# Decade-qiu/Go2NetSpectra

Hardware: AMD Instinct MI355X
Metric: Mpackets/s CMS update (device-resident, d=4 w=2^20) at 1/2/4/8 MI355X (higher is better)
Workload: dtype u32; 1 GPU; configs[1]: Count-Min d=4 w=2^20, 100M Zipf(1.1) 5-tuple headers in HBM per GPU, bit-exact counters; device_batch=100000000, key=5-tuple (37 B), parallelism=owner-key shards x1 (SrcIP slot; each GPU generates its shard of the stream), windows=steps use stream windows 0..619 (warmup first), none replayed

## Files before the change

go2netspectra_amd/_lib.py:

```python
from __future__ import annotations

import ctypes as ct
import os
import subprocess

_HERE = os.path.dirname(os.path.abspath(__file__))
LIB_PATH = os.environ.get("GNS_LIB") or os.path.join(_HERE, "libgns_sketch.so")
CSRC = os.path.join(_HERE, "csrc")

GNS_OK = 0
GNS_E_ARG, GNS_E_HIP, GNS_E_OOM, GNS_E_FULL, GNS_E_RANGE, GNS_E_NODEV = -1, -2, -3, -4, -5, -6
ERRORS = {-1: "GNS_E_ARG", -2: "GNS_E_HIP", -3: "GNS_E_OOM", -4: "GNS_E_FULL", -5: "GNS_E_RANGE",
          -6: "GNS_E_NODEV"}
MEM_HOST, MEM_DEVICE = 0, 1

FIELD_IDS = {"SrcIP": 1, "DstIP": 2, "SrcPort": 3, "DstPort": 4, "Protocol": 5}
FIELD_NAMES = {v: k for k, v in FIELD_IDS.items()}
FIELD_SIZE = {"SrcIP": 16, "DstIP": 16, "SrcPort": 2, "DstPort": 2, "Protocol": 1}

EXPORTED = [
    "gns_cm_create", "gns_cm_destroy", "gns_cm_insert_keys", "gns_cm_insert_tuples",
    "gns_cm_insert_headers", "gns_cm_flush", "gns_cm_query", "gns_cm_query_device", "gns_cm_heavy_hitters", "gns_cm_reset",
    "gns_cm_export_state", "gns_cm_stats", "gns_cm_counters", "gns_cm_set_timing", "gns_cm_stage_times", "gns_cm_stream",
    "gns_cm_view_create", "gns_cm_view_destroy", "gns_cm_view_refresh", "gns_cm_view_heavy_hitters",
    "gns_cm_view_query",
    "gns_ss_create", "gns_ss_destroy", "gns_ss_insert_keys", "gns_ss_insert_tuples",
    "gns_ss_insert_headers", "gns_ss_flush", "gns_ss_query", "gns_ss_query_device", "gns_ss_heavy_hitters", "gns_ss_reset",
    "gns_ss_export_state", "gns_ss_stats", "gns_ss_counters", "gns_ss_set_timing", "gns_ss_stage_times",
    "gns_synth_create", "gns_synth_destroy", "gns_synth_fill", "gns_synth_flows",
    "gns_ex_create", "gns_ex_destroy", "gns_ex_insert_tuples", "gns_ex_insert_headers", "gns_ex_flush",
    "gns_ex_query", "gns_ex_query_device", "gns_ex_snapshot", "gns_ex_reset", "gns_ex_counters", "gns_ex_set_timing",
    "gns_ex_stage_times",
    "gns_thrift_decode", "gns_pack_pcap", "gns_pack_pcap_ts", "gns_pack_counts", "gns_frame_record", "gns_last_error", "gns_version",
    "gns_route_create", "gns_route_destroy", "gns_route_partition",
    "gns_cm_dict_stats", "gns_ss_dict_stats", "gns_ex_dict_stats", "gns_cm_reclaim", "gns_ss_reclaim",
    "gns_cm_insert_compact", "gns_pack_pcap_compact", "gns_compact_headers", "gns_route_partition_async",
    "gns_pack_pcap_compact16", "gns_compact_headers16",
    "gns_route_owner_fields", "gns_route_create_keyed", "gns_route_owner_layout", "gns_route_owner_keys",
    "gns_device_alloc", "gns_device_free", "gns_cm_heavy_rows", "gns_hh_order_rows",
    "gns_exs_create", "gns_exs_destroy", "gns_exs_insert_keys", "gns_exs_insert_tuples", "gns_exs_insert_headers",
    "gns_exs_flush", "gns_exs_query", "gns_exs_query_device", "gns_exs_heavy_hitters", "gns_exs_snapshot",
    "gns_exs_reset", "gns_exs_counters", "gns_exs_dict_stats", "gns_exs_set_timing", "gns_exs_stage_times",
    "gns_ex_aggregate", "gns_ex_heavy_hitters",
    "gns_ex_view_create", "gns_ex_view_destroy", "gns_ex_view_refresh", "gns_ex_view_snapshot",
    "gns_ex_view_aggregate", "gns_ex_view_heavy_hitters",
    "gns_pairs_export", "gns_pairs_merge", "gns_pairs_merge_from",
    "gns_ss_insert_compact", "gns_spread_insert_compact", "gns_ex_insert_compact", "gns_pack_pcap_compact_ts",
    "gns_ss_view_create", "gns_ss_view_destroy", "gns_ss_view_refresh", "gns_ss_view_query",
    "gns_ss_view_query_device", "gns_ss_view_heavy_hitters", "gns_ss_view_heavy_rows", "gns_ss_view_export_state",
    "gns_cm_view_refresh_at", "gns_cm_view_query_device", "gns_cm_view_heavy_rows", "gns_cm_view_export_state",
    "gns_ex_rollup", "gns_spread_rollup",
    "gns_ex_rollup_prefix", "gns_spread_rollup_prefix", "gns_ex_aggregate_cidr", "gns_ex_view_aggregate_cidr",
    "gns_ex_hist_create", "gns_ex_hist_destroy", "gns_ex_hist_append", "gns_ex_hist_times", "gns_ex_hist_stats",
    "gns_ex_hist_aggregate", "gns_ex_hist_aggregate_cidr", "gns_ex_hist_heavy_hitters", "gns_ex_hist_snapshot",
    "gns_ex_hist_trim", "gns_ex_hist_export", "gns_ex_hist_append_rows",
    "gns_hh_hist_create", "gns_hh_hist_destroy", "gns_hh_hist_append", "gns_hh_hist_heavy_hitters",
    "gns_hh_hist_heavy_rows", "gns_hh_hist_times", "gns_hh_hist_stats", "gns_hh_hist_export",
]


class GnsError(RuntimeError):
    def __init__(self, code: int, msg: str):
        super().__init__(f"{ERRORS.get(code, code)}: {msg}")
        self.code = code


class Layout(ct.Structure):
    _fields_ = [("n_fields", ct.c_uint32), ("fields", ct.c_uint8 * 8)]

    @classmethod
    def of(cls, fields) -> "Layout":
        fields = list(fields or [])
        if len(fields) > 8:
            raise ValueError("at most 8 key fields")
        lay = cls()
        lay.n_fields = len(fields)
        for i, f in enumerate(fields):
            lay.fields[i] = FIELD_IDS.get(f, 0)
        return lay

    def names(self):
        return [FIELD_NAMES.get(int(self.fields[i]), "") for i in range(self.n_fields)]


class Tuples(ct.Structure):
    _fields_ = [("src16", ct.c_void_p), ("dst16", ct.c_void_p), ("sport", ct.c_void_p),
                ("dport", ct.c_void_p), ("proto", ct.c_void_p), ("length", ct.c_void_p)]


class CmParams(ct.Structure):
# ... 92 lines not shown
        "gns_cm_stream": ([vp], vp),
        "gns_cm_view_create": ([vp, vp], i32), "gns_cm_view_destroy": ([vp], i32),
        "gns_cm_view_refresh": ([vp], i32), "gns_cm_view_heavy_hitters": ([vp, vp, vp, vp, vp, vp, vp], i32),
        "gns_cm_view_query": ([vp, vp, u32, u64, vp], i32),
        "gns_ss_create": ([vp, vp], i32), "gns_ss_destroy": ([vp], i32),
        "gns_ss_insert_keys": ([vp, vp, u32, vp, u32, u64, i32], i32),
        "gns_ss_insert_tuples": ([vp, vp, u64, i32], i32),
        "gns_ss_insert_headers": ([vp, vp, vp, u64, i32], i32),
        "gns_ss_flush": ([vp], i32), "gns_ss_query": ([vp, vp, u32, u64, vp], i32),
        "gns_ss_query_device": ([vp, vp, u32, u64, vp], i32),
        "gns_ss_heavy_hitters": ([vp, vp, vp, vp], i32), "gns_ss_reset": ([vp], i32),
        "gns_ss_export_state": ([vp, vp, vp, vp, vp], i32), "gns_ss_stats": ([vp, vp], i32),
        "gns_ss_counters": ([vp, vp], i32),
        "gns_ss_set_timing": ([vp, i32], i32), "gns_ss_stage_times": ([vp, vp, vp, i32], i32),
        "gns_synth_create": ([vp, vp], i32), "gns_synth_destroy": ([vp], i32),
        "gns_synth_fill": ([vp, vp, vp, u64, u64], i32), "gns_synth_flows": ([vp, vp], i32),
        "gns_ex_create": ([vp, vp], i32), "gns_ex_destroy": ([vp], i32),
        "gns_ex_insert_tuples": ([vp, vp, vp, vp, u64, i32], i32),
        "gns_ex_insert_headers": ([vp, vp, vp, vp, u64, i32], i32),
        "gns_ex_flush": ([vp], i32), "gns_ex_query": ([vp, vp, u32, u64, vp], i32),
        "gns_ex_query_device": ([vp, vp, u32, u64, vp], i32),
        "gns_ex_snapshot": ([vp, vp, vp, vp, vp, vp, vp], i32), "gns_ex_reset": ([vp], i32),
        "gns_ex_counters": ([vp, vp], i32), "gns_ex_set_timing": ([vp, i32], i32),
        "gns_ex_stage_times": ([vp, vp, vp, i32], i32),
        "gns_thrift_decode": ([vp, u64, vp, u64, vp, vp, vp, vp, i32, i32], i32),
        "gns_pack_pcap": ([ct.c_char_p, vp, vp, u64, vp], ct.c_int64),
        "gns_pack_pcap_ts": ([ct.c_char_p, vp, vp, vp, u64, vp], ct.c_int64),
        "gns_pack_counts": ([vp], ct.c_int),
        "gns_frame_record": ([vp, ct.c_uint32, ct.c_uint32, vp], ct.c_int),
        "gns_last_error": ([], ct.c_char_p), "gns_version": ([], ct.c_char_p),
        "gns_route_create": ([u32, i32, vp], i32), "gns_route_destroy": ([vp], i32),
        "gns_route_partition": ([vp, vp, vp, u64, vp, vp, vp], i32),
        "gns_cm_dict_stats": ([vp, vp], i32), "gns_ss_dict_stats": ([vp, vp], i32),
        "gns_ex_dict_stats": ([vp, vp], i32), "gns_cm_reclaim": ([vp], i32), "gns_ss_reclaim": ([vp], i32),
        "gns_cm_insert_compact": ([vp, vp, vp, u64, vp, u64, i32], i32),
        "gns_pack_pcap_compact": ([ct.c_char_p, vp, vp, u64, vp, u64, vp, vp], ct.c_int64),
        "gns_compact_headers": ([vp, vp, u64, vp, vp, u64, vp, i32], i32),
        "gns_pack_pcap_compact16": ([ct.c_char_p, vp, u64, vp, u64, vp, vp], ct.c_int64),
        "gns_compact_headers16": ([vp, vp, u64, vp, vp, u64, vp, i32], i32),
        "gns_route_partition_async": ([vp, vp, vp, u64, vp, vp, vp, vp], i32),
        "gns_route_owner_fields": ([vp, u32, vp], i32),
        "gns_route_create_keyed": ([u32, vp, i32, vp], i32),
        "gns_route_owner_layout": ([vp, vp], i32),
        "gns_route_owner_keys": ([vp, vp, vp, u32, u64, vp, i32], i32),
        "gns_device_alloc": ([u64, i32, vp], i32), "gns_device_free": ([vp, i32], i32),
        "gns_cm_heavy_rows": ([vp, vp, vp, vp, vp], i32),
        "gns_hh_order_rows": ([vp, u32, u64, vp, i32], i32),
        "gns_exs_create": ([vp, vp], i32), "gns_exs_destroy": ([vp], i32),
        "gns_exs_insert_keys": ([vp, vp, u32, vp, u32, u64, i32], i32),
        "gns_exs_insert_tuples": ([vp, vp, u64, i32], i32),
        "gns_exs_insert_headers": ([vp, vp, vp, u64, i32], i32),
        "gns_exs_flush": ([vp], i32), "gns_exs_query": ([vp, vp, u32, u64, vp], i32),
        "gns_exs_query_device": ([vp, vp, u32, u64, vp], i32),
        "gns_exs_heavy_hitters": ([vp, u32, vp, vp, vp], i32), "gns_exs_snapshot": ([vp, vp, vp, vp], i32),
        "gns_exs_reset": ([vp], i32), "gns_exs_counters": ([vp, vp], i32), "gns_exs_dict_stats": ([vp, vp], i32),
        "gns_exs_set_timing": ([vp, i32], i32), "gns_exs_stage_times": ([vp, vp, vp, i32], i32),
        "gns_ex_aggregate": ([vp, vp, u32, vp], i32),
        "gns_ex_heavy_hitters": ([vp, i32, u64, u64, vp, vp, vp], i32),
        "gns_cm_import_state": ([vp, vp, vp, vp, vp, vp], i32),
        "gns_ss_import_state": ([vp, vp, vp, vp, vp, u64, vp], i32),
        "gns_ex_merge": ([vp, vp, vp, vp, vp, vp, u64, i32], i32),
        "gns_ex_rollup": ([vp, vp, vp], i32),
        "gns_spread_rollup": ([vp, vp, u64, vp, vp], i32),
        "gns_ex_rollup_prefix": ([vp, vp, vp, vp], i32),
        "gns_spread_rollup_prefix": ([vp, vp, vp, vp, u64, vp, vp], i32),
        "gns_ex_aggregate_cidr": ([vp, vp, u32, vp], i32),
# ... 113 lines not shown
```

go2netspectra_amd/csrc/gns_cm.hip:

```cpp
#include <algorithm>
#include <atomic>
#include <cstdlib>
#include <mutex>
#include <vector>

#include "gns_coldmask.cuh"
#include "gns_common.hpp"
#include "gns_ctl.cuh"
#include "gns_hh.hpp"
#include "gns_scan.cuh"
#include "gns_xcd.cuh"

namespace gns {

#ifndef GNS_TILE_BITS
#define GNS_TILE_BITS 12
#endif
#ifndef GNS_AP_THREADS
#define GNS_AP_THREADS 1024
#endif
#ifndef GNS_AP_ITEMS
#define GNS_AP_ITEMS 8
#endif
constexpr uint32_t kTileBitsMax = GNS_TILE_BITS;
// ... 2516 lines not shown
    uint32_t *C = nullptr, *S = nullptr, *Fc = nullptr, *Fs = nullptr;
    CmRead rd;
    std::atomic<uint32_t> period{0};
    std::mutex views_mu;
    std::vector<gns_cm_view *> views;
    uint32_t epoch = 0;
    uint64_t bmax = 0;
    uint32_t nblk_max = 0;
    uint32_t *keyid = nullptr, *idx = nullptr;
    uint64_t *cold = nullptr;
    uint64_t *pend[2] = {nullptr, nullptr};
    uint32_t *pcnt[2] = {nullptr, nullptr};
    uint32_t *ptotal = nullptr;
    uint32_t *hist = nullptr, *part = nullptr, *total = nullptr, *order = nullptr;
    uint64_t *entries = nullptr;
    uint64_t *ovf = nullptr;
    uint32_t *ovf_cnt = nullptr;
    uint64_t ovf_cap = 0;
    unsigned long long *stats = nullptr;
    uint32_t *hot_ids = nullptr;
    uint32_t *hot_tab = nullptr;
    long long *segtot = nullptr;
    uint32_t *hflag = nullptr, *hhist = nullptr, *hthr = nullptr, *hcnt = nullptr;
    uint32_t *hcand = nullptr, *hcn = nullptr;
    HotSum *hsum = nullptr;
    uint32_t *hflag2 = nullptr;
    uint32_t *work = nullptr;
    uint32_t ncu = 256;
    uint32_t *hres = nullptr;
    uint4 *chk = nullptr;
    bool warm = false;
    bool lds_ordered = false;
    uint32_t *h_pin = nullptr;
    HostStage stage[2];
    CompactInput compact;
    hipStream_t cstream = nullptr;
    hipEvent_t ev_copied[2] = {nullptr, nullptr}, ev_used[2] = {nullptr, nullptr};
    StageTimer timer;
};

enum : uint32_t { kViewPlain = 0, kViewDetached = 1 };
constexpr uint64_t kCmvPiece = 1u << 18;

struct gns_cm_view : ViewCore {
    gns_cm *cm = nullptr;
    uint32_t *C = nullptr, *S = nullptr, *Fc = nullptr, *Fs = nullptr;
    CmRead rd;
    uint32_t period = ~0u;
    std::atomic<uint32_t> kind{kViewPlain};
    DictDev T{};
    uint64_t tab_cap = 0;
    uint32_t *remap = nullptr;
    uint64_t remap_n = 0;
    uint32_t *scan = nullptr;
    uint64_t scan_n = 0;
    uint32_t *words = nullptr;
    unsigned long long *ctr = nullptr;
    uint8_t *xbytes = nullptr;
    uint64_t xbytes_n = 0;
    PinnedOut po;
    uint32_t *hsm = nullptr;
};

struct ViewsQuiesced {
    std::unique_lock<std::mutex> reg;
    std::vector<std::unique_lock<std::mutex>> locks;
    explicit ViewsQuiesced(gns_cm *cm) : reg(cm->views_mu) {
        locks.reserve(cm->views.size());
        for (gns_cm_view *v : cm->views)
            if (v->kind.load() != kViewDetached) locks.emplace_back(v->mu);
    }
};

namespace {

int cm_free_all(gns_cm *cm) {
    dfree(cm->C); dfree(cm->S); dfree(cm->Fc); dfree(cm->Fs); cm->rd.free_all();
    dfree(cm->keyid); dfree(cm->idx); dfree(cm->cold);
    dfree(cm->pend[0]); dfree(cm->pend[1]); dfree(cm->pcnt[0]); dfree(cm->pcnt[1]);
    dfree(cm->ptotal); dfree(cm->hist); dfree(cm->part); dfree(cm->total); dfree(cm->order);
    dfree(cm->entries); dfree(cm->ovf); dfree(cm->ovf_cnt); dfree(cm->stats);
    cm->stage[0].free_all(); cm->stage[1].free_all(); cm->compact.free_all();
    for (int i = 0; i < 2; i++) {
        if (cm->ev_copied[i]) (void)hipEventDestroy(cm->ev_copied[i]);
        if (cm->ev_used[i]) (void)hipEventDestroy(cm->ev_used[i]);
    }
    if (cm->cstream) (void)hipStreamDestroy(cm->cstream);
    dfree(cm->work);
    dfree(cm->hot_ids); dfree(cm->segtot); dfree(cm->hflag); dfree(cm->hhist); dfree(cm->hthr); dfree(cm->hcnt);
    dfree(cm->hcand); dfree(cm->hcn);
    dfree(cm->hsum); dfree(cm->hflag2); dfree(cm->hres); dfree(cm->chk); dfree(cm->hot_tab);
    cm->FlowDict::free_all();
    if (cm->h_pin) (void)hipHostFree(cm->h_pin);
    cm->timer.destroy();
    if (cm->stream) (void)hipStreamDestroy(cm->stream);
    return GNS_OK;
}

int cm_reset_state(gns_cm *cm) {
    const uint64_t cells = (uint64_t)cm->g.d * cm->g.w;
    GNS_HIP(hipMemsetAsync(cm->C, 0, cells * 4, cm->stream));
    GNS_HIP(hipMemsetAsync(cm->S, 0, cells * 4, cm->stream));
    GNS_HIP(hipMemsetAsync(cm->Fc, 0xFF, cells * 4, cm->stream));
    GNS_HIP(hipMemsetAsync(cm->Fs, 0xFF, cells * 4, cm->stream));
    GNS_HIP(hipMemsetAsync(cm->D.rec, 0, cm->dict_slots * cm->D.RW * 4, cm->stream));
    GNS_HIP(hipMemsetAsync(cm->hot_ids, 0xFF, (size_t)cm->g.d * kHot * 4, cm->stream));
    GNS_HIP(hipMemsetAsync(cm->hot_tab, 0xFF, (size_t)cm->g.d * kHotTab * 4, cm->stream));
    GNS_HIP(hipMemsetAsync(cm->hhist, 0, (size_t)cm->g.d * kHotKeys * 4, cm->stream));
    GNS_HIP(hipMemsetAsync(cm->hthr, 0xFF, 8 * 4, cm->stream));
    GNS_HIP(hipMemsetAsync(cm->hcn, 0, 16 * 4, cm->stream));
    GNS_HIP(hipMemsetAsync(cm->stats + 3, 0, 2 * sizeof(unsigned long long), cm->stream));
    GNS_HIP(hipMemsetAsync(cm->dctl, 0, 16, cm->stream));
    cm->claimed = 0;
    cm->full = false;
    cm->warm = false;
    return GNS_OK;
}

int cm_reclaim(gns_cm *cm, uint64_t min_slots = 0) {
    ViewsQuiesced q(cm);
    const uint64_t cells = (uint64_t)cm->g.d * cm->g.w;
    std::vector<DictIds> ids{{cm->Fc, cells}, {cm->Fs, cells}};
    const uint32_t period = cm->period.load();
    for (gns_cm_view *v : cm->views)
        if (v->kind.load() != kViewDetached && v->period == period) {
            ids.push_back({v->Fc, cells});
            ids.push_back({v->Fs, cells});
        }
    return cm->reclaim(ids.data(), (int)ids.size(), min_slots, cm->stream);
}

template <int KIND, int MODE>
int cm_run_batch(gns_cm *cm, const InputDesc &in, uint64_t n) {
    if (n == 0) return GNS_OK;
    hipStream_t s = cm->stream;
    const uint32_t nblk = (uint32_t)((n + kChunk - 1) / kChunk);
    const CmGeom &g = cm->g;
    ScopedStage total_stage(cm->timer, 5);
    {
        CtlZero z;
        z.add(cm->ptotal, 8);
        z.add(cm->dctl + 1, 4);
        z.add(cm->hflag2, ((size_t)g.d * kHot + 2) * 4);
        z.add(cm->stats + 8, 8);
        z.add(cm->ovf_cnt, 4);
        z.add(cm->work, 4);
        z.add(cm->hflag, (size_t)g.d * kHot * 4);
        GNS_HIP(ctl_zero(z, s));
// ... 5 lines not shown
        a.keyid = cm->keyid; a.idx = cm->idx; a.cold = cm->cold; a.pend = cm->pend[0]; a.pend_cnt = cm->pcnt[0];
        a.pend_total = cm->ptotal; a.hist = cm->hist; a.nblk = nblk; a.hot_ids = cm->hot_ids;
        a.Fc = cm->Fc; a.Fs = cm->Fs; a.hsum = cm->hsum; a.hot_tab = cm->hot_tab;
        a.stats = cm->stats;
        ScopedStage st(cm->timer, 0);
        const size_t lds = extract_lds_bytes(g.nbins_all, g.d);
        if constexpr (KIND == IN_REC16) {
            if (lds > kExLdsSmall)
                hipLaunchKernelGGL((k_extract<KIND, MODE, 0, 0, 1024>), dim3(nblk), dim3(1024), lds, s, a);
            else
                hipLaunchKernelGGL((k_extract<KIND, MODE, 0, 0, 256>), dim3(nblk), dim3(kExThreads), lds, s, a);
        } else if (lds > kExLdsSmall) {
            if (cm->K == 37 && g.d == 8)
                hipLaunchKernelGGL((k_extract<KIND, MODE, 37, 8, kC5Threads>), dim3(nblk), dim3(kC5Threads), lds, s, a);
            else if (cm->K == 37)
                hipLaunchKernelGGL((k_extract<KIND, MODE, 37, 0, 1024>), dim3(nblk), dim3(1024), lds, s, a);
            else if (cm->K == 16)
                hipLaunchKernelGGL((k_extract<KIND, MODE, 16, 0, 1024>), dim3(nblk), dim3(1024), lds, s, a);
            else
                hipLaunchKernelGGL((k_extract<KIND, MODE, 0, 0, 1024>), dim3(nblk), dim3(1024), lds, s, a);
        } else if (cm->K == 37 && g.d == 4)
            hipLaunchKernelGGL((k_extract<KIND, MODE, 37, 4, 256>), dim3(nblk), dim3(kExThreads), lds, s, a);
        else if (cm->K == 37)
            hipLaunchKernelGGL((k_extract<KIND, MODE, 37, 0, 256>), dim3(nblk), dim3(kExThreads), lds, s, a);
        else if (cm->K == 16 && g.d == 4)
            hipLaunchKernelGGL((k_extract<KIND, MODE, 16, 4, 256>), dim3(nblk), dim3(kExThreads), lds, s, a);
        else if (cm->K == 16)
            hipLaunchKernelGGL((k_extract<KIND, MODE, 16, 0, 256>), dim3(nblk), dim3(kExThreads), lds, s, a);
        else
            hipLaunchKernelGGL((k_extract<KIND, MODE, 0, 0, 256>), dim3(nblk), dim3(kExThreads), lds, s, a);
        GNS_HIP(hipGetLastError());
    }
    int cur = 0;
    for (int round = 0;; round++) {
        if (round > 1) {
            CtlRead rd;
            rd.add(cm->ptotal + cur, 4, 0);
            rd.add(cm->stats + 3, 8, 2);
            rd.add(cm->dctl, 4, 4);
            if (round == 2) rd.add(cm->stats + 8, 8, 6);
            GNS_HIP(ctl_read(rd, cm->h_pin, s));
            GNS_HIP(hipStreamSynchronize(s));
            cm->claimed = cm->h_pin[4];
            if (round == 2) {
                const uint64_t big = (uint64_t)cm->h_pin[6] | (uint64_t)cm->h_pin[7] << 32;
                if (big * g.d > cm->ovf_cap) {
                    const uint64_t want = std::min<uint64_t>(std::max<uint64_t>(big * g.d + big * g.d / 4, kOvfCap), 1ull << 31);
                    dfree(cm->ovf);
                    cm->ovf = nullptr;
                    cm->ovf_cap = 0;
                    GNS_TRY(dalloc_t(&cm->ovf, want));
                    cm->ovf_cap = want;
                }
            }
            if (cm->h_pin[2] | cm->h_pin[3]) {
                set_error("flow dictionary full (%llu slots); raise max_flows",
                          (unsigned long long)cm->dict_slots);
                return GNS_E_FULL;
            }
            if (cm->h_pin[0] == 0) break;
        }
        if (round > 64) { set_error("dictionary resolve did not converge"); return GNS_E_FULL; }
        if (++cm->epoch == 0) cm->epoch = 1;
        ResolveArgs a{};
        a.in = in; a.n = n; a.kp = cm->kp; a.D = cm->D; a.epoch = cm->epoch; a.keyid = cm->keyid;
        a.pend_in = cm->pend[cur]; a.cnt_in = cm->pcnt[cur];
        a.pend_out = cm->pend[cur ^ 1]; a.cnt_out = cm->pcnt[cur ^ 1]; a.total_out = cm->ptotal + (cur ^ 1);
        a.total_in = cm->ptotal + cur;
        a.stats = cm->stats; a.g = g;
        ScopedStage st(cm->timer, 1);
        hipLaunchKernelGGL((k_resolve<KIND, MODE>), dim3(nblk), dim3(kExThreads), 0, s, a);
        GNS_HIP(hipGetLastError());
        cur ^= 1;
    }
    {
        ScopedStage st(cm->timer, 2);
        const uint32_t ngrp = (nblk + kTGrp - 1) / kTGrp;
        const dim3 g2((g.nbins_all + 255) / 256, ngrp);
        uint32_t *tot = cm->part + (size_t)ngrp * g.nbins_all;
        hipLaunchKernelGGL(k_tscan_part, g2, dim3(256), 0, s, cm->hist, nblk, g.nbins_all, cm->part);
        hipLaunchKernelGGL(k_tscan_mid, dim3((g.nbins_all + 255) / 256), dim3(256), 0, s, cm->part, ngrp, g.nbins_all, tot);
        hipLaunchKernelGGL(k_tscan_bins, dim3(1), dim3(1024), 0, s, tot, g.nbins_all, cm->total);
        hipLaunchKernelGGL(k_tscan_down, g2, dim3(256), 0, s, cm->hist, nblk, g.nbins_all, cm->part, tot);
        GNS_HIP(hipGetLastError());
    }
    {
        ScatterArgs a{};
        a.n = n; a.g = g; a.keyid = cm->keyid; a.idx = cm->idx; a.sizes = in.sizes;
        a.offsets = cm->hist; a.nblk = nblk; a.entries = cm->entries; a.ovf = cm->ovf; a.cold = cm->cold;
        a.ovf_cnt = cm->ovf_cnt; a.ovf_cap = (uint32_t)cm->ovf_cap; a.hot_ids = cm->hot_ids; a.stats = cm->stats;
        a.hot_mode = 0; a.hflag2 = cm->hflag2; a.hany = cm->hflag2 + g.d * kHot;
        ScopedStage st(cm->timer, 3);
        if (cm->lds_ordered && g.ntiles <= 256)
            hipLaunchKernelGGL((k_scatter_st<256, false>), dim3(nblk), dim3(kStThreads), 0, s, a);
        else if (cm->lds_ordered && g.ntiles <= 512)
            hipLaunchKernelGGL((k_scatter_st<512, true>), dim3(nblk), dim3(kStThreads), 0, s, a);
        else if (cm->lds_ordered)
            hipLaunchKernelGGL(k_scatter<1>, dim3(nblk), dim3(kScThreads), scatter_lds_bytes(g.ntiles + kHot, g.d), s, a);
        else
            hipLaunchKernelGGL(k_scatter<0>, dim3(nblk), dim3(kScThreads), scatter_lds_bytes(g.ntiles + kHot, g.d), s, a);
        GNS_HIP(hipGetLastError());
    }
    {
        const bool ordered = g.nbins <= 4096;
        if (ordered)
            hipLaunchKernelGGL(k_order, dim3(1), dim3(1024), 0, s, cm->hist, nblk, g.nbins, g.nbins_all,
                               cm->total, cm->order);
        ApplyArgs a{};
        a.stats = cm->stats;
        a.entries = cm->entries; a.offsets = cm->hist; a.nblk = nblk; a.nbins = g.nbins;
        a.total = cm->total; a.order = ordered ? cm->order : nullptr; a.ovf = cm->ovf; a.g = g;
        a.C = cm->C; a.Fc = cm->Fc; a.S = cm->S; a.Fs = cm->Fs; a.work = cm->work;
        ScopedStage st(cm->timer, 4);
        if (g.sub_bits) {
            const dim3 apg(std::min(g.nbins, cm->ncu));
            hipLaunchKernelGGL(k_apply_sparse, apg, dim3(kApThreads), 0, s, a);
        } else {
            const dim3 apg(std::min(g.nbins, cm->ncu * (kApThreads <= 512 ? 2u : 1u)));
            hipLaunchKernelGGL(k_apply, apg, dim3(kApThreads), 0, s, a);
        }
        GNS_HIP(hipGetLastError());
    }
    {
        HotArgs h{};
        h.entries = cm->entries; h.offsets = cm->hist; h.nblk = nblk; h.total = cm->total; h.ovf = cm->ovf;
        h.hot_ids = cm->hot_ids; h.g = g; h.C = cm->C; h.Fc = cm->Fc; h.S = cm->S; h.Fs = cm->Fs;
        h.segtot = cm->segtot; h.hflag = cm->hflag;
        h.hsum = cm->hsum; h.hflag2 = cm->hflag2; h.hany = cm->hflag2 + g.d * kHot; h.nchk = h.hany + 1;
        h.hres = cm->hres; h.chk = cm->chk; h.chk_cap = kChkCap;
        h.keyid = cm->keyid; h.idx = cm->idx; h.sizes = in.sizes; h.n = n;
        ScopedStage st(cm->timer, 6);
        hipLaunchKernelGGL(k_hot_decide, dim3(g.d * kHot), dim3(256), 0, s, h);
        hipLaunchKernelGGL(k_hot_blockcheck, dim3(kChkCap), dim3(256), 0, s, h);
        hipLaunchKernelGGL(k_hot_commit, dim3((g.d * kHot + 511) / 512), dim3(512), 0, s, h);
        {
            ScatterArgs a{};
            a.n = n; a.g = g; a.keyid = cm->keyid; a.idx = cm->idx; a.sizes = in.sizes;
            a.offsets = cm->hist; a.nblk = nblk; a.entries = cm->entries; a.ovf = cm->ovf;
            a.ovf_cnt = cm->ovf_cnt; a.ovf_cap = (uint32_t)cm->ovf_cap; a.hot_ids = cm->hot_ids; a.stats = cm->stats;
            a.hot_mode = 1; a.hflag2 = cm->hflag2; a.hany = h.hany;
            if (cm->lds_ordered)
                hipLaunchKernelGGL(k_scatter<1>, dim3(nblk), dim3(kScThreads), scatter_lds_bytes(g.ntiles + kHot, g.d), s, a);
            else
                hipLaunchKernelGGL(k_scatter<0>, dim3(nblk), dim3(kScThreads), scatter_lds_bytes(g.ntiles + kHot, g.d), s, a);
        }
        hipLaunchKernelGGL(k_hot_sum, dim3(1024), dim3(256), 0, s, h);
        hipLaunchKernelGGL(k_hot_verify, dim3(1024), dim3(256), 0, s, h);
        hipLaunchKernelGGL(k_hot_apply, dim3((g.d * kHot + 511) / 512), dim3(512), 0, s, h);
        hipLaunchKernelGGL(k_hot_fallback, dim3(g.d * kHot), dim3(64), 0, s, h);
        GNS_HIP(hipGetLastError());
    }
    {
        ScopedStage st(cm->timer, 7);
        const unsigned grid = (unsigned)std::min<uint64_t>(2048, ((uint64_t)g.w / 4 + 255) / 256 + 1);
        uint32_t *hcn = cm->hcn, *hfull = cm->hcn + 8;
        hipLaunchKernelGGL(k_hot_hist, dim3(std::min(grid, 512u)), dim3(256), 0, s, cm->C, g, cm->hhist, cm->hthr,
                           cm->hcand, hcn);
        hipLaunchKernelGGL(k_hot_pick, dim3(1), dim3(512), 0, s, cm->hhist, g, cm->hthr, cm->hcnt, cm->hot_ids, hcn,
                           hfull);
        hipLaunchKernelGGL(k_hot_collect, dim3(grid), dim3(256), 0, s, cm->C, g, cm->hthr, cm->hcnt, cm->hot_ids,
                           cm->hcand, hcn, hfull);
        hipLaunchKernelGGL(k_hot_table, dim3(1), dim3(1024), 0, s, g, cm->hot_ids, cm->hot_tab, hcn);
        GNS_HIP(hipGetLastError());
    }
    cm->warm = true;
    return GNS_OK;
}

template <int KIND>
int cm_batch(gns_cm *cm, const InputDesc &d, uint64_t m) {
    if constexpr (KIND == IN_KEYS) {
        return cm_run_batch<KIND, PLAN_SLICE0>(cm, d, m);
    } else {
        switch (plan_mode(cm->kp)) {
        case PLAN_SLICE0: return cm_run_batch<KIND, PLAN_SLICE0>(cm, d, m);
        case PLAN_SLICE4: return cm_run_batch<KIND, PLAN_SLICE4>(cm, d, m);
        default: return cm_run_batch<KIND, PLAN_GENERIC>(cm, d, m);
        }
    }
}

template <int KIND>
int cm_batch_recover(gns_cm *cm, const InputDesc &d, uint64_t m) {
    static const std::string piece = std::to_string(kChunk) + "-packet batch";
    const DictRecovery r{*cm, cm->stats, cm->stream, kChunk, piece.c_str(),
                         [cm](const InputDesc &pd, uint64_t pm) { return cm_batch<KIND>(cm, pd, pm); },
                         [cm](uint64_t min_slots) { return cm_reclaim(cm, min_slots); }};
    return r.batch(d, m, false);
}

int stage_host_batch(gns_cm *cm, int b, const InputDesc &in, uint64_t off, uint64_t m, InputDesc &d) {
    if (!cm->cstream) {
        GNS_HIP(hipStreamCreateWithFlags(&cm->cstream, hipStreamNonBlocking));
        for (int i = 0; i < 2; i++) {
            GNS_HIP(hipEventCreateWithFlags(&cm->ev_copied[i], hipEventDisableTiming));
            GNS_HIP(hipEventCreateWithFlags(&cm->ev_used[i], hipEventDisableTiming));
        }
    }
    StageList l;
    d = advance(in, off);
    stage_input(l, d, m);
    if (in.rec_len) stage_add<uint32_t>(l, nullptr, m * 4, &d.sizes);
    HostStage &sg = cm->stage[b];
    if (sg.cap < HostStage::need(l)) GNS_HIP(hipEventSynchronize(cm->ev_used[b]));
    GNS_HIP(hipStreamWaitEvent(cm->cstream, cm->ev_used[b], 0));
    GNS_TRY(sg.copy(l, cm->cstream));
    if (in.rec_len) GNS_TRY(CompactInput::unpack_sizes_into(d.rec16, m, const_cast<uint32_t *>(d.sizes), cm->cstream));
    if (d.keys) d.aligned = (d.stride % 4 == 0 && d.stride >= ((cm->K + 3) & ~3u)) ? 1u : 0u;
    GNS_HIP(hipEventRecord(cm->ev_copied[b], cm->cstream));
    return GNS_OK;
}

template <int KIND>
int cm_insert(gns_cm *cm, InputDesc in, uint64_t n, gns_mem where) {
    GNS_TRY(set_device(cm->device));
    auto batch_len = [&](uint64_t off, bool warm) {
        const uint64_t m = std::min<uint64_t>(cm->bmax, n - off);
        return warm ? m : std::min<uint64_t>(m, std::max<uint64_t>(kChunk * 64, cm->bmax / 32));
    };
// ... 109 lines not shown
        cm->D.bw = cm->D.RW >= 16 && 1 + (cm->K + 3) / 4 <= 12 ? 1u : 0u;
        cm->D.seed = 0x2545F491u;
        if ((rc = dalloc_t(&cm->D.rec, slots * cm->D.RW)) != GNS_OK) break;
        if ((rc = dalloc_t(&cm->dctl, 4)) != GNS_OK || (rc = dalloc_t(&cm->stats_bak, 3)) != GNS_OK) break;
        cm->D.ctl = cm->dctl;
        cm->limits();
        cm->bmax = p->batch_packets ? p->batch_packets : (16ull << 20);
        cm->bmax = ((cm->bmax + kChunk - 1) / kChunk) * kChunk;
        if (cm->bmax > (1ull << 31)) { set_error("batch_packets too large"); rc = GNS_E_ARG; break; }
        const uint64_t bcap = (((1ull << 31) / g.d) / kChunk) * kChunk;
        if (cm->bmax > bcap) cm->bmax = bcap;
        cm->nblk_max = (uint32_t)(cm->bmax / kChunk);
        const uint64_t nscan = ((uint64_t)(cm->nblk_max + kTGrp - 1) / kTGrp + 2) * g.nbins_all;
        if ((rc = dalloc_t(&cm->keyid, cm->bmax)) || (rc = dalloc_t(&cm->idx, cm->bmax * g.d)) ||
            (rc = dalloc_t(&cm->cold, cm->bmax / 64)) ||
            (rc = dalloc_t(&cm->pend[0], cm->bmax)) || (rc = dalloc_t(&cm->pend[1], cm->bmax)) ||
            (rc = dalloc_t(&cm->pcnt[0], cm->nblk_max)) || (rc = dalloc_t(&cm->pcnt[1], cm->nblk_max)) ||
            (rc = dalloc_t(&cm->ptotal, 2)) || (rc = dalloc_t(&cm->hist, (uint64_t)g.nbins_all * cm->nblk_max)) ||
            (rc = dalloc_t(&cm->part, nscan)) || (rc = dalloc_t(&cm->total, 1)) ||
            (rc = dalloc_t(&cm->order, g.nbins)) || (rc = dalloc_t(&cm->entries, cm->bmax * g.d)) ||
            (rc = dalloc_t(&cm->ovf, kOvfCap)) || (rc = dalloc_t(&cm->ovf_cnt, 1)) ||
            (rc = dalloc_t(&cm->stats, kStatsProf + 16)) || (rc = dalloc_t(&cm->work, 1)) || (rc = dalloc_t(&cm->hot_ids, g.d * kHot)) ||
            (rc = dalloc_t(&cm->segtot, (size_t)g.d * kHot * kHotSegs * 2)) || (rc = dalloc_t(&cm->hflag, g.d * kHot)) ||
            (rc = dalloc_t(&cm->hhist, g.d * kHotKeys)) || (rc = dalloc_t(&cm->hthr, 8)) || (rc = dalloc_t(&cm->hcnt, 8)) ||
            (rc = dalloc_t(&cm->hcand, (size_t)g.d * kHotCand)) || (rc = dalloc_t(&cm->hcn, 16)) ||
            (rc = dalloc_t(&cm->hsum, (uint64_t)g.d * kHot * cm->nblk_max)) ||
            (rc = dalloc_t(&cm->hflag2, g.d * kHot + 2)) || (rc = dalloc_t(&cm->hres, g.d * kHot * 2)) ||
            (rc = dalloc_t(&cm->chk, kChkCap)) || (rc = dalloc_t(&cm->hot_tab, (size_t)g.d * kHotTab)))
            break;
        cm->ovf_cap = kOvfCap;
        if (hipHostMalloc(reinterpret_cast<void **>(&cm->h_pin), 64, 0) != hipSuccess) {
            set_error("hipHostMalloc failed"); rc = GNS_E_OOM; break;
        }
        if (hipMemsetAsync(cm->stats, 0, (kStatsProf + 16) * 8, cm->stream) != hipSuccess) { rc = GNS_E_HIP; break; }
        if ((rc = cm_reset_state(cm)) != GNS_OK) break;
        {
            const char *env = getenv("GNS_K3_RANK");
            uint32_t *viol = nullptr;
            if ((rc = dalloc_t(&viol, 1)) != GNS_OK) break;
            hipError_t e = hipMemsetAsync(viol, 0, 4, cm->stream);
            if (e == hipSuccess) {
                hipLaunchKernelGGL(k_lds_order_probe, dim3(4 * cm->ncu), dim3(256), 0, cm->stream, viol, 64);
                e = hipGetLastError();
            }
            uint32_t hv = 1;
            if (e == hipSuccess) e = hipMemcpyAsync(&hv, viol, 4, hipMemcpyDeviceToHost, cm->stream);
            if (e == hipSuccess) e = hipStreamSynchronize(cm->stream);
            dfree(viol);
            if (e != hipSuccess) { set_error("lds order probe: %s", hipGetErrorString(e)); rc = GNS_E_HIP; break; }
            cm->lds_ordered = hv == 0 && !(env && env[0] == '0');
        }
        if ((rc = hh_reserve(cm->rd.hh, (uint64_t)cm->g.d * cm->g.w, cm->dict_slots, cm->K, cm->stream)) != GNS_OK) break;
        if (hipStreamSynchronize(cm->stream) != hipSuccess) { set_error("sync failed"); rc = GNS_E_HIP; break; }
    } while (0);
    if (rc != GNS_OK) {
        cm_free_all(cm);
        delete cm;
        return rc;
    }
    *out = cm;
    return GNS_OK;
}

int gns_cm_destroy(gns_cm *cm) {
    if (!cm) return GNS_OK;
    (void)hipSetDevice(cm->device);
// ... 490 lines not shown
#if defined(GNS_SP_PROF)
    for (int i = 0; i < 7; i++) out[i] = h[kStatsProf + i];
    out[7] = h[6];
    return GNS_OK;
#endif
#ifdef GNS_K3_PROF
    for (int i = 0; i < 8; i++) out[i] = h[kStatsProf + i];
    return GNS_OK;
#endif
#ifdef GNS_K4_PROF
    for (int i = 0; i < 4; i++) out[i] = h[kStatsProf + i];
    out[4] = h[kStatsProf + 9];
    out[5] = h[kStatsProf + 5];
    out[6] = h[kStatsProf + 8];
    out[7] = h[kStatsProf + 6];
#else
    for (int i = 0; i < 8; i++) out[i] = h[i];
#endif
    return GNS_OK;
}

int gns_cm_reclaim(gns_cm *cm) {
    if (!cm) return GNS_E_ARG;
    GNS_TRY(set_device(cm->device));
    return cm_reclaim(cm);
}

int gns_cm_dict_stats(gns_cm *cm, uint64_t out[8]) {
    if (!cm || !out) return GNS_E_ARG;
    cm->FlowDict::stats(out);
    return GNS_OK;
}

int gns_cm_set_timing(gns_cm *cm, int on) {
    if (!cm) return GNS_E_ARG;
    set_timing_arg(cm->timer, on);
    return GNS_OK;
}

int gns_cm_stage_times(gns_cm *cm, double ms[8], uint64_t launches[8], int reset) {
    if (!cm) return GNS_E_ARG;
    GNS_TRY(set_device(cm->device));
    cm->timer.report(ms, launches, reset);
    return GNS_OK;
}

void *gns_cm_stream(gns_cm *cm) { return cm ? (void *)cm->stream : nullptr; }

}
```

go2netspectra_amd/csrc/gns_ctl.cuh:

```cuda
#pragma once
#include <hip/hip_runtime.h>
#include <cstdint>

namespace gns {
namespace {

constexpr int kCtlMax = 16;

struct CtlZero {
    uint32_t *p[kCtlMax];
    uint32_t n[kCtlMax];
    int k = 0;
    void add(void *ptr, size_t bytes) { p[k] = static_cast<uint32_t *>(ptr); n[k] = (uint32_t)(bytes / 4); k++; }
};

__global__ __launch_bounds__(256) void k_ctl_zero(CtlZero z) {
    for (int i = 0; i < z.k; i++)
        for (uint32_t j = threadIdx.x; j < z.n[i]; j += 256) z.p[i][j] = 0u;
}

struct CtlRead {
    const uint32_t *src[kCtlMax];
    uint32_t at[kCtlMax];
    int k = 0;
    void add(const void *ptr, size_t bytes, uint32_t word) {
        for (uint32_t w = 0; w < bytes / 4; w++) {
            src[k] = static_cast<const uint32_t *>(ptr) + w;
            at[k] = word + w;
            k++;
        }
    }
};

__global__ __launch_bounds__(64) void k_ctl_read(CtlRead r, uint32_t *dst) {
    const int i = (int)threadIdx.x;
    if (i < r.k) dst[r.at[i]] = *r.src[i];
}

inline hipError_t ctl_zero(const CtlZero &z, hipStream_t s) {
    hipLaunchKernelGGL(k_ctl_zero, dim3(1), dim3(256), 0, s, z);
    return hipGetLastError();
}

inline hipError_t ctl_read(const CtlRead &r, uint32_t *dst_pinned, hipStream_t s) {
    hipLaunchKernelGGL(k_ctl_read, dim3(1), dim3(64), 0, s, r, dst_pinned);
    return hipGetLastError();
}

}
}
```

go2netspectra_amd/sketch.py:

```python
from __future__ import annotations

import ctypes as ct
from dataclasses import dataclass, field
from typing import List, Optional, Sequence

import numpy as np

from . import _lib
from ._lib import check


@dataclass
class HeavySize:
    Flow: bytes
    Size: int


@dataclass
class HeavyCount:
    Flow: bytes
    Count: int


@dataclass
# ... 300 lines not shown
        Fc = np.empty((n, K), np.uint8)
        Fs = np.empty((n, K), np.uint8)
        check(self._L.gns_cm_export_state(self._h, C.ctypes.data, S.ctypes.data, Fc.ctypes.data,
                                          Fs.ctypes.data))
        return C, S, Fc[:, : self.key_bytes], Fs[:, : self.key_bytes]

    def import_state(self, C, S, FPc, FPs, counters=None) -> None:
        n = self.depth * self.width
        C, S = _host(C, np.uint32).reshape(-1), _host(S, np.uint32).reshape(-1)
        FPc, FPs = _host(FPc, np.uint8).reshape(-1), _host(FPs, np.uint8).reshape(-1)
        if C.size != n or S.size != n or FPc.size != n * self.key_bytes or FPs.size != n * self.key_bytes:
            raise ValueError(f"import_state: arrays do not match {self.depth} x {self.width} cells of "
                             f"{self.key_bytes}-byte keys")
        cnt = None if counters is None else _host(counters, np.uint64).reshape(-1)
        if cnt is not None and cnt.size < 3:
            raise ValueError("import_state: counters needs 3 values")
        check(self._L.gns_cm_import_state(self._h, C.ctypes.data, S.ctypes.data, FPc.ctypes.data, FPs.ctypes.data,
                                          None if cnt is None else cnt.ctypes.data))

    def stats(self) -> dict:
        s = (ct.c_uint64 * 4)()
        check(self._L.gns_cm_stats(self._h, s))
        return {"inserted": s[0], "dropped": s[1], "unsupported": s[2], "flows": s[3]}

    def counters(self) -> dict:
        c = (ct.c_uint64 * 8)()
        check(self._L.gns_cm_counters(self._h, c))
        names = ["inserted", "dropped", "unsupported", "dict_full", "ovf_full", "replayed", "chunks",
                 "chunks_replay"]
        return dict(zip(names, list(c)))

    def dict_stats(self) -> dict:
        return _lib.dict_stats(self._L.gns_cm_dict_stats, self._h)

    def reclaim(self) -> None:
        check(self._L.gns_cm_reclaim(self._h))

    def set_timing(self, on: bool = True, stages=None) -> None:
        check(self._L.gns_cm_set_timing(self._h, _lib.timing_arg(on, stages, self.STAGES)))

    STAGES = ["extract", "resolve", "scan", "scatter", "apply", "insert", "hot", "designate"]

    def stage_times(self, reset: bool = False) -> dict:
        ms = (ct.c_double * 8)()
        ln = (ct.c_uint64 * 8)()
        check(self._L.gns_cm_stage_times(self._h, ms, ln, 1 if reset else 0))
        return {name: (ms[i], ln[i]) for i, name in enumerate(self.STAGES)}

    def stream(self) -> int:
        return int(self._L.gns_cm_stream(self._h) or 0)


def _ss_heavy_arrays(fn, h, flow_bytes, owner):
    K = max(flow_bytes, 1)
    hint = getattr(owner, "_hh_cap", 0)
    while True:
        cap = max(hint, 1)
        f = np.empty((cap, K), np.uint8)
        v = np.empty(cap, np.uint32)
        n = ct.c_uint64(cap)
        check(fn(h, f.ctypes.data, v.ctypes.data, ct.byref(n)))
        if n.value <= cap:
            owner._hh_cap = 2 * n.value + 64
            return f[: n.value, : flow_bytes], v[: n.value]
        hint = n.value

# ... 259 lines not shown
```

include/gns_sketch.h:

```cpp
#ifndef GNS_SKETCH_H
#define GNS_SKETCH_H
#include <stddef.h>
#include <stdint.h>

#ifdef __cplusplus
extern "C" {
#endif

typedef enum gns_status {
    GNS_OK = 0,
    GNS_E_ARG = -1,
    GNS_E_HIP = -2,
    GNS_E_OOM = -3,
    GNS_E_FULL = -4,
    GNS_E_RANGE = -5,
    GNS_E_NODEV = -6
} gns_status;

typedef enum gns_mem { GNS_MEM_HOST = 0, GNS_MEM_DEVICE = 1 } gns_mem;

#define GNS_TIMING_MASK 0x100

typedef enum gns_field {
    GNS_F_NONE = 0, GNS_F_SRCIP = 1, GNS_F_DSTIP = 2, GNS_F_SRCPORT = 3, GNS_F_DSTPORT = 4,
// ... 21 lines not shown
    uint32_t size_threshold, count_threshold;
    gns_layout flow;
    uint32_t key_bytes;
    const uint32_t *seeds;
    uint64_t max_flows;
    uint64_t batch_packets;
    int device;
    uint32_t bucket_lo, bucket_hi;
} gns_cm_params;

int gns_cm_create(const gns_cm_params *p, gns_cm **out);
int gns_cm_destroy(gns_cm *cm);
int gns_cm_insert_keys(gns_cm *cm, const uint8_t *keys, uint32_t stride, const uint32_t *sizes,
                       uint64_t n, gns_mem where);
int gns_cm_insert_tuples(gns_cm *cm, const gns_tuples *t, uint64_t n, gns_mem where);
int gns_cm_insert_headers(gns_cm *cm, const uint8_t *hdr, const uint32_t *wirelen, uint64_t n,
                          gns_mem where);
int gns_cm_insert_compact(gns_cm *cm, const uint8_t *rec16, const uint32_t *wirelen, uint64_t n,
                          const uint8_t *side64, uint64_t n_side, gns_mem where);
int gns_cm_flush(gns_cm *cm);
int gns_cm_query(gns_cm *cm, const uint8_t *keys, uint32_t stride, uint64_t n, uint64_t *out);
int gns_cm_query_device(gns_cm *cm, const uint8_t *keys, uint32_t stride, uint64_t n, uint64_t *out);
int gns_cm_heavy_hitters(gns_cm *cm, uint8_t *count_flows, uint32_t *counts, uint64_t *n_count,
                         uint8_t *size_flows, uint32_t *sizes, uint64_t *n_size);
int gns_cm_heavy_rows(gns_cm *cm, uint8_t *count_rows, uint64_t *n_count, uint8_t *size_rows, uint64_t *n_size);
int gns_hh_order_rows(const uint8_t *rows, uint32_t key_bytes, uint64_t n, uint8_t *out_rows, int device);
int gns_cm_reset(gns_cm *cm);
int gns_cm_export_state(gns_cm *cm, uint32_t *C, uint32_t *S, uint8_t *FPc, uint8_t *FPs);
int gns_cm_import_state(gns_cm *cm, const uint32_t *C, const uint32_t *S, const uint8_t *FPc, const uint8_t *FPs,
                        const uint64_t *counters );
int gns_cm_stats(gns_cm *cm, uint64_t stats[4]);
int gns_cm_counters(gns_cm *cm, uint64_t out[8]);
int gns_cm_dict_stats(gns_cm *cm, uint64_t out[8]);
int gns_cm_reclaim(gns_cm *cm);
int gns_cm_set_timing(gns_cm *cm, int on);
int gns_cm_stage_times(gns_cm *cm, double ms[8], uint64_t launches[8], int reset);
void *gns_cm_stream(gns_cm *cm);

typedef struct gns_cm_view gns_cm_view;
int gns_cm_view_create(gns_cm *cm, gns_cm_view **out);
int gns_cm_view_destroy(gns_cm_view *v);
int gns_cm_view_refresh(gns_cm_view *v);
int gns_cm_view_heavy_hitters(gns_cm_view *v, uint8_t *count_flows, uint32_t *counts, uint64_t *n_count,
                              uint8_t *size_flows, uint32_t *sizes, uint64_t *n_size);
int gns_cm_view_query(gns_cm_view *v, const uint8_t *keys, uint32_t stride, uint64_t n, uint64_t *out);

#define GNS_CM_VIEW_DETACH 1u
int gns_cm_view_refresh_at(gns_cm_view *v, uint32_t flags);
int gns_cm_view_query_device(gns_cm_view *v, const uint8_t *keys, uint32_t stride, uint64_t n, uint64_t *out);
int gns_cm_view_heavy_rows(gns_cm_view *v, uint8_t *count_rows, uint64_t *n_count, uint8_t *size_rows,
                           uint64_t *n_size);
int gns_cm_view_export_state(gns_cm_view *v, uint32_t *C, uint32_t *S, uint8_t *FPc, uint8_t *FPs,
                             uint64_t *counters );

typedef struct gns_ss gns_ss;

typedef struct gns_ss_params {
    uint32_t width, depth, threshold;
    uint32_t m, size;
    double base, b;
    gns_layout flow, elem;
    uint32_t flow_bytes, elem_bytes;
    const uint32_t *seeds;
    uint64_t hll_master;
    uint64_t rng_seed;
    uint64_t batch_packets;
// ... 242 lines not shown
```

Baseline: 22620 Mpackets/s.

## Overlap dictionary-resolve checks with scan and hot decide; skip exact hot path when unneeded

Runs two dictionary resolve rounds speculatively, then records an event instead of synchronizing the stream. The scan, order and hot-decide kernels are queued before the host waits on the control readback. The hot decision is read back asynchronously, and the exact hot-path kernels (second scatter, sum, verify, apply, fallback) now launch only when the hot flag says they are needed. It adds counters and a debug entry point, a system fence in the control-read kernel, and a redecide path for when resolve takes more than two rounds.

Result: no change. 22650 Mpackets/s, median of 2 (+0.2%).

```diff
diff --git a/go2netspectra_amd/_lib.py b/go2netspectra_amd/_lib.py
--- a/go2netspectra_amd/_lib.py
+++ b/go2netspectra_amd/_lib.py
@@ -56,6 +56,7 @@
     "gns_ex_hist_trim", "gns_ex_hist_export", "gns_ex_hist_append_rows",
     "gns_hh_hist_create", "gns_hh_hist_destroy", "gns_hh_hist_append", "gns_hh_hist_heavy_hitters",
     "gns_hh_hist_heavy_rows", "gns_hh_hist_times", "gns_hh_hist_stats", "gns_hh_hist_export",
+    "gns_cm_debug_tail",
 ]
 
 
@@ -214,6 +215,7 @@
         "gns_route_create": ([u32, i32, vp], i32), "gns_route_destroy": ([vp], i32),
         "gns_route_partition": ([vp, vp, vp, u64, vp, vp, vp], i32),
         "gns_cm_dict_stats": ([vp, vp], i32), "gns_ss_dict_stats": ([vp, vp], i32),
+        "gns_cm_debug_tail": ([vp, vp, vp], i32),
         "gns_ex_dict_stats": ([vp, vp], i32), "gns_cm_reclaim": ([vp], i32), "gns_ss_reclaim": ([vp], i32),
         "gns_cm_insert_compact": ([vp, vp, vp, u64, vp, u64, i32], i32),
         "gns_pack_pcap_compact": ([ct.c_char_p, vp, vp, u64, vp, u64, vp, vp], ct.c_int64),
diff --git a/go2netspectra_amd/csrc/gns_cm.hip b/go2netspectra_amd/csrc/gns_cm.hip
--- a/go2netspectra_amd/csrc/gns_cm.hip
+++ b/go2netspectra_amd/csrc/gns_cm.hip
@@ -2572,6 +2572,8 @@
     bool warm = false;
     bool lds_ordered = false;
     uint32_t *h_pin = nullptr;
+    hipEvent_t ev_chk = nullptr, ev_hany = nullptr;
+    uint64_t n_batch = 0, n_exact = 0, n_redecide = 0, n_retried = 0;
     HostStage stage[2];
     CompactInput compact;
     hipStream_t cstream = nullptr;
@@ -2629,6 +2631,8 @@
     dfree(cm->work);
     dfree(cm->hot_ids); dfree(cm->segtot); dfree(cm->hflag); dfree(cm->hhist); dfree(cm->hthr); dfree(cm->hcnt);
     dfree(cm->hcand); dfree(cm->hcn);
+    if (cm->ev_chk) (void)hipEventDestroy(cm->ev_chk);
+    if (cm->ev_hany) (void)hipEventDestroy(cm->ev_hany);
     dfree(cm->hsum); dfree(cm->hflag2); dfree(cm->hres); dfree(cm->chk); dfree(cm->hot_tab);
     cm->FlowDict::free_all();
     if (cm->h_pin) (void)hipHostFree(cm->h_pin);
@@ -2654,6 +2658,7 @@
     cm->claimed = 0;
     cm->full = false;
     cm->warm = false;
+    cm->n_batch = cm->n_exact = cm->n_redecide = cm->n_retried = 0;
     return GNS_OK;
 }
 
@@ -2725,35 +2730,7 @@
         GNS_HIP(hipGetLastError());
     }
     int cur = 0;
-    for (int round = 0;; round++) {
-        if (round > 1) {
-            CtlRead rd;
-            rd.add(cm->ptotal + cur, 4, 0);
-            rd.add(cm->stats + 3, 8, 2);
-            rd.add(cm->dctl, 4, 4);
-            if (round == 2) rd.add(cm->stats + 8, 8, 6);
-            GNS_HIP(ctl_read(rd, cm->h_pin, s));
-            GNS_HIP(hipStreamSynchronize(s));
-            cm->claimed = cm->h_pin[4];
-            if (round == 2) {
-                const uint64_t big = (uint64_t)cm->h_pin[6] | (uint64_t)cm->h_pin[7] << 32;
-                if (big * g.d > cm->ovf_cap) {
-                    const uint64_t want = std::min<uint64_t>(std::max<uint64_t>(big * g.d + big * g.d / 4, kOvfCap), 1ull << 31);
-                    dfree(cm->ovf);
-                    cm->ovf = nullptr;
-                    cm->ovf_cap = 0;
-                    GNS_TRY(dalloc_t(&cm->ovf, want));
-                    cm->ovf_cap = want;
-                }
-            }
-            if (cm->h_pin[2] | cm->h_pin[3]) {
-                set_error("flow dictionary full (%llu slots); raise max_flows",
-                          (unsigned long long)cm->dict_slots);
-                return GNS_E_FULL;
-            }
-            if (cm->h_pin[0] == 0) break;
-        }
-        if (round > 64) { set_error("dictionary resolve did not converge"); return GNS_E_FULL; }
+    auto resolve_round = [&]() -> int {
         if (++cm->epoch == 0) cm->epoch = 1;
         ResolveArgs a{};
         a.in = in; a.n = n; a.kp = cm->kp; a.D = cm->D; a.epoch = cm->epoch; a.keyid = cm->keyid;
@@ -2765,7 +2742,38 @@
         hipLaunchKernelGGL((k_resolve<KIND, MODE>), dim3(nblk), dim3(kExThreads), 0, s, a);
         GNS_HIP(hipGetLastError());
         cur ^= 1;
-    }
+        return GNS_OK;
+    };
+    auto read_checks = [&](bool first) -> int {
+        CtlRead rd;
+        rd.add(cm->ptotal + cur, 4, 0);
+        rd.add(cm->stats + 3, 8, 2);
+        rd.add(cm->dctl, 4, 4);
+        if (first) rd.add(cm->stats + 8, 8, 6);
+        return ctl_read(rd, cm->h_pin, s) == hipSuccess ? GNS_OK : GNS_E_HIP;
+    };
+    HotArgs h{};
+    h.offsets = cm->hist; h.nblk = nblk; h.total = cm->total;
+    h.hot_ids = cm->hot_ids; h.g = g; h.C = cm->C; h.Fc = cm->Fc; h.S = cm->S; h.Fs = cm->Fs;
+    h.segtot = cm->segtot; h.hflag = cm->hflag;
+    h.hsum = cm->hsum; h.hflag2 = cm->hflag2; h.hany = cm->hflag2 + g.d * kHot; h.nchk = h.hany + 1;
+    h.hres = cm->hres; h.chk = cm->chk; h.chk_cap = kChkCap;
+    h.keyid = cm->keyid; h.idx = cm->idx; h.sizes = in.sizes; h.n = n;
+    auto decide = [&]() -> int {
+        ScopedStage st(cm->timer, 6);
+        hipLaunchKernelGGL(k_hot_decide, dim3(g.d * kHot), dim3(256), 0, s, h);
+        hipLaunchKernelGGL(k_hot_blockcheck, dim3(kChkCap), dim3(256), 0, s, h);
+        GNS_HIP(hipGetLastError());
+        CtlRead rd;
+        rd.add(h.hany, 4, 12);
+        GNS_HIP(ctl_read(rd, cm->h_pin, s));
+        GNS_HIP(hipEventRecord(cm->ev_hany, s));
+        return GNS_OK;
+    };
+    GNS_TRY(resolve_round());
+    GNS_TRY(resolve_round());
+    GNS_TRY(read_checks(true));
+    GNS_HIP(hipEventRecord(cm->ev_chk, s));
     {
         ScopedStage st(cm->timer, 2);
         const uint32_t ngrp = (nblk + kTGrp - 1) / kTGrp;
@@ -2776,6 +2784,47 @@
         hipLaunchKernelGGL(k_tscan_bins, dim3(1), dim3(1024), 0, s, tot, g.nbins_all, cm->total);
         hipLaunchKernelGGL(k_tscan_down, g2, dim3(256), 0, s, cm->hist, nblk, g.nbins_all, cm->part, tot);
         GNS_HIP(hipGetLastError());
+    }
+    const bool ordered = g.nbins <= 4096;
+    if (ordered) {
+        hipLaunchKernelGGL(k_order, dim3(1), dim3(1024), 0, s, cm->hist, nblk, g.nbins, g.nbins_all,
+                           cm->total, cm->order);
+        GNS_HIP(hipGetLastError());
+    }
+    GNS_TRY(decide());
+    GNS_HIP(hipEventSynchronize(cm->ev_chk));
+    cm->claimed = cm->h_pin[4];
+    {
+        const uint64_t big = (uint64_t)cm->h_pin[6] | (uint64_t)cm->h_pin[7] << 32;
+        if (big * g.d > cm->ovf_cap) {
+            const uint64_t want = std::min<uint64_t>(std::max<uint64_t>(big * g.d + big * g.d / 4, kOvfCap), 1ull << 31);
+            dfree(cm->ovf);
+            cm->ovf = nullptr;
+            cm->ovf_cap = 0;
+            GNS_TRY(dalloc_t(&cm->ovf, want));
+            cm->ovf_cap = want;
+        }
+    }
+    auto dict_full = [&]() -> bool {
+        if (!(cm->h_pin[2] | cm->h_pin[3])) return false;
+        set_error("flow dictionary full (%llu slots); raise max_flows", (unsigned long long)cm->dict_slots);
+        return true;
+    };
+    if (dict_full()) return GNS_E_FULL;
+    if (cm->h_pin[0] != 0) {
+        for (int round = 2; cm->h_pin[0] != 0; round++) {
+            if (round > 64) { set_error("dictionary resolve did not converge"); return GNS_E_FULL; }
+            GNS_TRY(resolve_round());
+            GNS_TRY(read_checks(false));
+            GNS_HIP(hipStreamSynchronize(s));
+            cm->claimed = cm->h_pin[4];
+            if (dict_full()) return GNS_E_FULL;
+        }
+        CtlZero z;
+        z.add(cm->hflag2, ((size_t)g.d * kHot + 2) * 4);
+        GNS_HIP(ctl_zero(z, s));
+        GNS_TRY(decide());
+        cm->n_redecide++;
     }
     {
         ScatterArgs a{};
@@ -2795,10 +2844,6 @@
         GNS_HIP(hipGetLastError());
     }
     {
-        const bool ordered = g.nbins <= 4096;
-        if (ordered)
-            hipLaunchKernelGGL(k_order, dim3(1), dim3(1024), 0, s, cm->hist, nblk, g.nbins, g.nbins_all,
-                               cm->total, cm->order);
         ApplyArgs a{};
         a.stats = cm->stats;
         a.entries = cm->entries; a.offsets = cm->hist; a.nblk = nblk; a.nbins = g.nbins;
@@ -2815,18 +2860,13 @@
         GNS_HIP(hipGetLastError());
     }
     {
-        HotArgs h{};
-        h.entries = cm->entries; h.offsets = cm->hist; h.nblk = nblk; h.total = cm->total; h.ovf = cm->ovf;
-        h.hot_ids = cm->hot_ids; h.g = g; h.C = cm->C; h.Fc = cm->Fc; h.S = cm->S; h.Fs = cm->Fs;
-        h.segtot = cm->segtot; h.hflag = cm->hflag;
-        h.hsum = cm->hsum; h.hflag2 = cm->hflag2; h.hany = cm->hflag2 + g.d * kHot; h.nchk = h.hany + 1;
-        h.hres = cm->hres; h.chk = cm->chk; h.chk_cap = kChkCap;
-        h.keyid = cm->keyid; h.idx = cm->idx; h.sizes = in.sizes; h.n = n;
+        GNS_HIP(hipEventSynchronize(cm->ev_hany));
+        const bool exact = cm->h_pin[12] != 0;
+        h.entries = cm->entries; h.ovf = cm->ovf;
         ScopedStage st(cm->timer, 6);
-        hipLaunchKernelGGL(k_hot_decide, dim3(g.d * kHot), dim3(256), 0, s, h);
-        hipLaunchKernelGGL(k_hot_blockcheck, dim3(kChkCap), dim3(256), 0, s, h);
         hipLaunchKernelGGL(k_hot_commit, dim3((g.d * kHot + 511) / 512), dim3(512), 0, s, h);
-        {
+        if (exact) {
+            cm->n_exact++;
             ScatterArgs a{};
             a.n = n; a.g = g; a.keyid = cm->keyid; a.idx = cm->idx; a.sizes = in.sizes;
             a.offsets = cm->hist; a.nblk = nblk; a.entries = cm->entries; a.ovf = cm->ovf;
@@ -2836,11 +2876,11 @@
                 hipLaunchKernelGGL(k_scatter<1>, dim3(nblk), dim3(kScThreads), scatter_lds_bytes(g.ntiles + kHot, g.d), s, a);
             else
                 hipLaunchKernelGGL(k_scatter<0>, dim3(nblk), dim3(kScThreads), scatter_lds_bytes(g.ntiles + kHot, g.d), s, a);
-        }
-        hipLaunchKernelGGL(k_hot_sum, dim3(1024), dim3(256), 0, s, h);
-        hipLaunchKernelGGL(k_hot_verify, dim3(1024), dim3(256), 0, s, h);
-        hipLaunchKernelGGL(k_hot_apply, dim3((g.d * kHot + 511) / 512), dim3(512), 0, s, h);
-        hipLaunchKernelGGL(k_hot_fallback, dim3(g.d * kHot), dim3(64), 0, s, h);
+            hipLaunchKernelGGL(k_hot_sum, dim3(1024), dim3(256), 0, s, h);
+            hipLaunchKernelGGL(k_hot_verify, dim3(1024), dim3(256), 0, s, h);
+            hipLaunchKernelGGL(k_hot_apply, dim3((g.d * kHot + 511) / 512), dim3(512), 0, s, h);
+            hipLaunchKernelGGL(k_hot_fallback, dim3(g.d * kHot), dim3(64), 0, s, h);
+        }
         GNS_HIP(hipGetLastError());
     }
     {
@@ -2856,6 +2896,7 @@
         hipLaunchKernelGGL(k_hot_table, dim3(1), dim3(1024), 0, s, g, cm->hot_ids, cm->hot_tab, hcn);
         GNS_HIP(hipGetLastError());
     }
+    cm->n_batch++;
     cm->warm = true;
     return GNS_OK;
 }
@@ -2877,7 +2918,11 @@
 int cm_batch_recover(gns_cm *cm, const InputDesc &d, uint64_t m) {
     static const std::string piece = std::to_string(kChunk) + "-packet batch";
     const DictRecovery r{*cm, cm->stats, cm->stream, kChunk, piece.c_str(),
-                         [cm](const InputDesc &pd, uint64_t pm) { return cm_batch<KIND>(cm, pd, pm); },
+                         [cm](const InputDesc &pd, uint64_t pm) {
+                             const int rc = cm_batch<KIND>(cm, pd, pm);
+                             if (rc == GNS_E_FULL && !cm->full) cm->n_retried++;
+                             return rc;
+                         },
                          [cm](uint64_t min_slots) { return cm_reclaim(cm, min_slots); }};
     return r.batch(d, m, false);
 }
@@ -3053,6 +3098,10 @@
         if (hipHostMalloc(reinterpret_cast<void **>(&cm->h_pin), 64, 0) != hipSuccess) {
             set_error("hipHostMalloc failed"); rc = GNS_E_OOM; break;
         }
+        if (hipEventCreateWithFlags(&cm->ev_chk, hipEventDisableTiming) != hipSuccess ||
+            hipEventCreateWithFlags(&cm->ev_hany, hipEventDisableTiming) != hipSuccess) {
+            set_error("hipEventCreate failed"); rc = GNS_E_HIP; break;
+        }
         if (hipMemsetAsync(cm->stats, 0, (kStatsProf + 16) * 8, cm->stream) != hipSuccess) { rc = GNS_E_HIP; break; }
         if ((rc = cm_reset_state(cm)) != GNS_OK) break;
         {
@@ -3609,6 +3658,17 @@
     return GNS_OK;
 }
 
+int gns_cm_debug_tail(gns_cm *cm, uint64_t out[4], uint32_t *hot_ids) {
+    if (!cm || !out) return GNS_E_ARG;
+    out[0] = cm->n_batch; out[1] = cm->n_exact; out[2] = cm->n_redecide; out[3] = cm->n_retried;
+    if (hot_ids) {
+        GNS_TRY(set_device(cm->device));
+        GNS_HIP(hipMemcpyAsync(hot_ids, cm->hot_ids, (size_t)cm->g.d * kHot * 4, hipMemcpyDeviceToHost, cm->stream));
+        GNS_HIP(hipStreamSynchronize(cm->stream));
+    }
+    return GNS_OK;
+}
+
 int gns_cm_set_timing(gns_cm *cm, int on) {
     if (!cm) return GNS_E_ARG;
     set_timing_arg(cm->timer, on);
diff --git a/go2netspectra_amd/csrc/gns_ctl.cuh b/go2netspectra_amd/csrc/gns_ctl.cuh
--- a/go2netspectra_amd/csrc/gns_ctl.cuh
+++ b/go2netspectra_amd/csrc/gns_ctl.cuh
@@ -35,6 +35,7 @@
 __global__ __launch_bounds__(64) void k_ctl_read(CtlRead r, uint32_t *dst) {
     const int i = (int)threadIdx.x;
     if (i < r.k) dst[r.at[i]] = *r.src[i];
+    __threadfence_system();
 }
 
 inline hipError_t ctl_zero(const CtlZero &z, hipStream_t s) {
diff --git a/go2netspectra_amd/sketch.py b/go2netspectra_amd/sketch.py
--- a/go2netspectra_amd/sketch.py
+++ b/go2netspectra_amd/sketch.py
@@ -356,6 +356,15 @@
 
     def dict_stats(self) -> dict:
         return _lib.dict_stats(self._L.gns_cm_dict_stats, self._h)
+
+    def debug_tail(self, hot_ids: bool = False) -> dict:
+        c = (ct.c_uint64 * 4)()
+        ids = np.empty((self.depth, 128), np.uint32) if hot_ids else None
+        check(self._L.gns_cm_debug_tail(self._h, c, ids.ctypes.data if hot_ids else None))
+        out = dict(zip(["batches", "exact", "redecided", "retried"], list(c)))
+        if hot_ids:
+            out["hot_ids"] = ids
+        return out
 
     def reclaim(self) -> None:
         check(self._L.gns_cm_reclaim(self._h))
diff --git a/include/gns_sketch.h b/include/gns_sketch.h
--- a/include/gns_sketch.h
+++ b/include/gns_sketch.h
@@ -77,6 +77,7 @@
 int gns_cm_stats(gns_cm *cm, uint64_t stats[4]);
 int gns_cm_counters(gns_cm *cm, uint64_t out[8]);
 int gns_cm_dict_stats(gns_cm *cm, uint64_t out[8]);
+int gns_cm_debug_tail(gns_cm *cm, uint64_t out[4], uint32_t *hot_ids);
 int gns_cm_reclaim(gns_cm *cm);
 int gns_cm_set_timing(gns_cm *cm, int on);
 int gns_cm_stage_times(gns_cm *cm, double ms[8], uint64_t launches[8], int reset);
```
